# a-slide/Quade

Hardware: AMD Instinct MI355X
Metric: read-pairs/sec demultiplexed (2x150 bp, dual 8 bp index) (higher is better)
Workload: dtype u8

## Files before the change

quade_amd/csrc/quade_deflate.hip:

```cpp
#include <hip/hip_runtime.h>
#include <stdint.h>
#include <stdio.h>

#include "crc_lds.h"
#include "quade_deflate.h"

namespace {
constexpr int BLOCK = 256, TILE = BLOCK * 16;
constexpr uint32_t HEADER_BITS = 80 + 3 + 14 + 19 * 3 + 259 * 4;

__device__ uint32_t rev_bits(uint32_t v, int n) { return __brev(v) >> (32 - n); }

__device__ void code_lengths(const uint32_t* freq, int n, uint8_t* len, uint16_t* order , uint32_t* w , int16_t* parent ) {
    int m = 0;
    for (int s = 0; s < n; ++s) {
        len[s] = 0;
        if (freq[s]) order[m++] = (uint16_t)s;
    }
    for (int s = 0; m < 2 && s < n; ++s) {
        bool used = false;
        for (int i = 0; i < m; ++i) used |= order[i] == s;
        if (!used) order[m++] = (uint16_t)s;
    }
    auto f = [&](int s) -> uint32_t { return freq[s] ? freq[s] : 1u; };
    for (int i = 1; i < m; ++i) {
        const uint16_t s = order[i];
        int j = i - 1;
        while (j >= 0 && (f(order[j]) > f(s) || (f(order[j]) == f(s) && order[j] > s))) {
            order[j + 1] = order[j];
            --j;
        }
        order[j + 1] = s;
    }
    for (int i = 0; i < m; ++i) w[i] = f(order[i]);
    for (int i = 0; i < 2 * m - 1; ++i) parent[i] = -1;
    int leaf = 0, inner = m, next = m;
    while (next < 2 * m - 1) {
        int pick[2];
        for (int k = 0; k < 2; ++k) pick[k] = (leaf < m && (inner >= next || w[leaf] <= w[inner])) ? leaf++ : inner++;
        w[next] = w[pick[0]] + w[pick[1]];
        parent[pick[0]] = parent[pick[1]] = (int16_t)next;
        ++next;
    }
    int bl[16] = {0};
    w[2 * m - 2] = 0;
    for (int k = 2 * m - 3; k >= 0; --k) w[k] = w[parent[k]] + 1;
    for (int i = 0; i < m; ++i) ++bl[w[i] < 15 ? w[i] : 15];
    uint32_t kraft = 0;
    for (int d = 1; d <= 15; ++d) kraft += (uint32_t)bl[d] << (15 - d);
    for (uint32_t excess = kraft - (1u << 15); excess > 0; --excess) {
        int bits = 14;
        while (bl[bits] == 0) --bits;
        --bl[bits];
        bl[bits + 1] += 2;
        --bl[15];
    }
    int at = 0;
    for (int bits = 15; bits >= 1; --bits)
        for (int c = 0; c < bl[bits]; ++c) len[order[at++]] = (uint8_t)bits;
}

__global__ __launch_bounds__(BLOCK) void huff_pieces(const uint8_t* text, const qd_deflate_piece* pieces, uint8_t* out,
                                                     int64_t out_stride, uint32_t* out_bytes) {
    __shared__ uint32_t hist[4][4][256];
    __shared__ uint32_t freq[257];
    __shared__ uint32_t lut[257];
    __shared__ uint8_t len[257];
    __shared__ uint16_t order[257];
    __shared__ uint32_t wtmp[513];
    __shared__ int16_t parent[513];
    __shared__ uint32_t scan[BLOCK];
    __shared__ uint32_t words[TILE * 15 / 32 + 16];
    __shared__ uint32_t carry_word, carry_bits;
    const int tid = threadIdx.x, wave = tid >> 6, rep = tid & 3;
    const int64_t a = (int64_t)pieces[blockIdx.x].text_off, L = (int64_t)pieces[blockIdx.x].text_len;
    const uint8_t* src = text + a;
    uint32_t* dst = reinterpret_cast<uint32_t*>(out + (int64_t)blockIdx.x * out_stride);
    for (int i = tid; i < 4 * 4 * 256; i += BLOCK) (&hist[0][0][0])[i] = 0;
    __syncthreads();
    for (int64_t t = 0; t < L; t += TILE) {
        const int64_t p = t + (int64_t)tid * 16;
        if (p + 16 <= L) {
            const uint4 v = *reinterpret_cast<const uint4*>(src + p);
            const uint32_t q[4] = {v.x, v.y, v.z, v.w};
#pragma unroll
            for (int j = 0; j < 16; ++j) atomicAdd(&hist[wave][rep][(q[j >> 2] >> (8 * (j & 3))) & 0xff], 1u);
        } else {
            for (int64_t i = p; i < L; ++i) atomicAdd(&hist[wave][rep][src[i]], 1u);
        }
    }
    __syncthreads();
    for (int s = tid; s < 256; s += BLOCK) {
        uint32_t c = 0;
        for (int i = 0; i < 16; ++i) c += (&hist[0][0][0])[i * 256 + s];
        freq[s] = c;
    }
    if (tid == 0) freq[256] = 1;
    __syncthreads();
    if (tid == 0) {
        code_lengths(freq, 257, len, order, wtmp, parent);
        int blc[16] = {0}, nxt[16] = {0};
        for (int s = 0; s < 257; ++s) ++blc[len[s]];
        blc[0] = 0;
        for (int b = 1, c = 0; b <= 15; ++b) {
            c = (c + blc[b - 1]) << 1;
            nxt[b] = c;
        }
        for (int s = 0; s < 257; ++s) lut[s] = len[s] ? ((uint32_t)len[s] | (rev_bits((uint32_t)nxt[len[s]]++, len[s]) << 8)) : 0;
        uint64_t acc = 0;
        int cnt = 0, wi = 0;
        auto put = [&](uint32_t v, int n) {
            acc |= (uint64_t)v << cnt;
            cnt += n;
            if (cnt >= 32) {
                dst[wi++] = (uint32_t)acc;
                acc >>= 32;
                cnt -= 32;
            }
        };
        const uint8_t head[10] = {0x1f, 0x8b, 8, 0, 0, 0, 0, 0, 0, 0xff};
        for (int i = 0; i < 10; ++i) put(head[i], 8);
        put(1, 1);
        put(2, 2);
        put(0, 5);
        put(1, 5);
        put(15, 4);
        const uint8_t ord[19] = {16, 17, 18, 0, 8, 7, 9, 6, 10, 5, 11, 4, 12, 3, 13, 2, 14, 1, 15};
        for (int k = 0; k < 19; ++k) put(ord[k] < 16 ? 4 : 0, 3);
        for (int s = 0; s < 257; ++s) put(rev_bits(len[s], 4), 4);
        put(rev_bits(1, 4), 4);
        put(rev_bits(1, 4), 4);
        carry_word = (uint32_t)acc;
        carry_bits = (uint32_t)cnt;
        scan[0] = (uint32_t)wi;
        uint64_t bits = HEADER_BITS;
        for (int s = 0; s < 257; ++s) bits += (uint64_t)freq[s] * len[s];
        scan[1] = ((bits + 7) / 8 + 8 + 8 <= (uint64_t)out_stride) ? 1u : 0u;
    }
    __syncthreads();
    uint32_t out_word = scan[0];
    const bool fits = scan[1] != 0;
    __syncthreads();
    if (!fits) {
        if (tid == 0) out_bytes[blockIdx.x] = 0;
        return;
    }
    for (int64_t t = 0; t < L; t += TILE) {
        const int64_t p = t + (int64_t)tid * 16;
        uint32_t q[4] = {0, 0, 0, 0};
        int nbytes = 0;
        if (p + 16 <= L) {
            const uint4 v = *reinterpret_cast<const uint4*>(src + p);
            q[0] = v.x; q[1] = v.y; q[2] = v.z; q[3] = v.w;
            nbytes = 16;
        } else if (p < L) {
            nbytes = (int)(L - p);
            for (int i = 0; i < nbytes; ++i) q[i >> 2] |= (uint32_t)src[p + i] << (8 * (i & 3));
        }
        uint64_t b[4] = {0, 0, 0, 0};
        uint32_t nb = 0;
#pragma unroll
        for (int j = 0; j < 16; ++j) {
            if (j < nbytes) {
                const uint32_t e = lut[(q[j >> 2] >> (8 * (j & 3))) & 0xff];
                const uint64_t c = e >> 8;
                const uint32_t l = e & 0xff, wi = nb >> 6, sh = nb & 63;
                b[wi] |= c << sh;
                if (sh + l > 64 && wi < 3) b[wi + 1] |= c >> (64 - sh);
                nb += l;
            }
        }
        uint32_t x = nb;
#pragma unroll
        for (int d = 1; d < 64; d <<= 1) {
            const uint32_t y = __shfl_up(x, d, 64);
            if ((tid & 63) >= d) x += y;
        }
        if ((tid & 63) == 63) scan[wave] = x;
        __syncthreads();
        uint32_t base = 0, total = 0;
#pragma unroll
        for (int i = 0; i < BLOCK / 64; ++i) {
            const uint32_t v = scan[i];
            if (i < wave) base += v;
            total += v;
        }
        const uint32_t mine = base + x - nb;
        const uint32_t cb = carry_bits, cw = carry_word;
        const uint32_t nwords = (cb + total + 31) >> 5;
        for (uint32_t i = tid; i <= nwords; i += BLOCK) words[i] = i == 0 ? cw : 0;
        __syncthreads();
        if (nb) {
            const uint32_t pos = cb + mine, w0 = pos >> 5, sh = pos & 31;
            uint32_t prev = 0;
#pragma unroll
            for (int i = 0; i < 8; ++i) {
                const uint32_t d = (uint32_t)(b[i >> 1] >> (32 * (i & 1)));
                const uint32_t o = sh ? (d << sh) | (prev >> (32 - sh)) : d;
                if (o && 32u * i < nb + sh) atomicOr(&words[w0 + i], o);
                prev = d;
            }
            const uint32_t o = sh ? prev >> (32 - sh) : 0;
            if (o) atomicOr(&words[w0 + 8], o);
        }
        __syncthreads();
        const uint32_t full = (cb + total) >> 5;
        for (uint32_t i = tid; i < full; i += BLOCK) dst[out_word + i] = words[i];
        __syncthreads();
        if (tid == 0) {
            carry_word = words[full];
            carry_bits = (cb + total) & 31;
        }
        out_word += full;
        __syncthreads();
    }
    if (tid == 0) {
        uint64_t acc = carry_word;
        int cnt = (int)carry_bits;
        const uint32_t e = lut[256];
        acc |= (uint64_t)(e >> 8) << cnt;
        cnt += (int)(e & 0xff);
        uint8_t* bytes = reinterpret_cast<uint8_t*>(dst) + (size_t)out_word * 4;
        int nby = 0;
        while (cnt > 0) {
            bytes[nby++] = (uint8_t)acc;
            acc >>= 8;
            cnt -= 8;
        }
        const uint32_t c = pieces[blockIdx.x].crc32, isz = (uint32_t)L;
        for (int i = 0; i < 4; ++i) bytes[nby++] = (uint8_t)(c >> (8 * i));
        for (int i = 0; i < 4; ++i) bytes[nby++] = (uint8_t)(isz >> (8 * i));
        out_bytes[blockIdx.x] = out_word * 4 + (uint32_t)nby;
    }
}

}

hipError_t qd_launch_huffman(const uint8_t* text, const qd_deflate_piece* pieces, uint32_t n_pieces, uint8_t* out, int64_t out_stride,
                             uint32_t* out_bytes, hipStream_t st) {
    if (n_pieces == 0) return hipSuccess;
    hipLaunchKernelGGL(huff_pieces, dim3(n_pieces), dim3(BLOCK), 0, st, text, pieces, out, out_stride, out_bytes);
    return hipGetLastError();
}

namespace {
#ifndef QD_LZ_WAVES
#define QD_LZ_WAVES 8
#endif
constexpr int LZ_SUB = QD_LZ_SUB, LZ_WAVES = QD_LZ_WAVES, LZ_BLOCK = 64 * LZ_WAVES, LZ_REG = LZ_SUB / LZ_WAVES;
constexpr int LZ_HASH_BITS = 11, LZ_NICE = 32, LZ_DNA_MIN = 12, LZ_MATCH_BITS = 13, LZ_MAXLEN = 256;
constexpr int LZ_CRC_SW = LZ_WAVES >= 16 ? 17 : (LZ_WAVES >= 8 ? 33 : 65);
constexpr int LZ_TEXT_WORDS = (LZ_SUB + 320) / 4;
constexpr int LZ_NL = 286, LZ_ND = 30;
static_assert(LZ_SUB <= 65536 && LZ_SUB % 256 == 0, "table entries are 16-bit positions inside the sub-block");

__device__ __forceinline__ uint32_t rd32(const uint32_t* tw, uint32_t p) {
    const uint32_t i = p >> 2;
    return __builtin_amdgcn_alignbyte(tw[i + 1], tw[i], p & 3u);
}
__device__ __forceinline__ void rd256(const uint32_t* tw, uint32_t p, uint32_t (&a)[8]) {
    const uint32_t i = p >> 2, sh = p & 3u;
    uint32_t w[9];
#pragma unroll
    for (int k = 0; k < 9; ++k) w[k] = tw[i + k];
#pragma unroll
    for (int k = 0; k < 8; ++k) a[k] = __builtin_amdgcn_alignbyte(w[k + 1], w[k], sh);
}
__device__ __forceinline__ uint32_t same32(const uint32_t* tw, const uint32_t (&a)[8], uint32_t c) {
    uint32_t b[8];
    rd256(tw, c, b);
    uint32_t n = 32;
#pragma unroll
    for (int k = 7; k >= 0; --k) {
        const uint32_t x = a[k] ^ b[k];
        if (x) n = 4u * (uint32_t)k + ((uint32_t)__builtin_ctz(x) >> 3);
    }
    return n;
}
__device__ __forceinline__ bool bases4(uint32_t v) {
    return __builtin_amdgcn_perm(0x4E000000u, 0x47544341u, (v >> 1) & 0x07070707u) == v;
}
__device__ __forceinline__ void len_symbol(uint32_t l, uint32_t& sym, uint32_t& eb, uint32_t& ev) {
    if (l < 8) {
        sym = 257 + l;
        eb = ev = 0;
    } else if (l == 255) {
        sym = 285;
        eb = ev = 0;
    } else {
        const uint32_t n = 31u - (uint32_t)__clz(l);
        eb = n - 2;
        sym = 257 + 4 * (n - 1) + ((l >> eb) & 3u);
        ev = l & ((1u << eb) - 1);
    }
}
__device__ __forceinline__ void dist_symbol(uint32_t d, uint32_t& sym, uint32_t& eb, uint32_t& ev) {
    if (d < 4) {
        sym = d;
        eb = ev = 0;
    } else {
        const uint32_t n = 31u - (uint32_t)__clz(d);
        eb = n - 1;
        sym = 2 * n + ((d >> eb) & 1u);
        ev = d & ((1u << eb) - 1);
    }
}
__device__ __forceinline__ uint32_t len_extra_bits(uint32_t sym) {
    return (sym < 265 || sym == 285) ? 0u : (sym - 261) >> 2;
}
__device__ __forceinline__ uint32_t dist_extra_bits(uint32_t sym) { return sym < 4 ? 0u : (sym >> 1) - 1; }

__device__ void block_code_lengths(const uint32_t* freq, int n, uint8_t* len, uint32_t* fx, uint16_t* order, uint32_t* w, int16_t* parent,
                                   uint32_t* m_out) {
    __shared__ uint32_t bl[16];
    const int tid = threadIdx.x, nthr = blockDim.x;
    for (int s = tid; s < n; s += nthr) {
        fx[s] = freq[s];
        len[s] = 0;
    }
    if (tid < 16) bl[tid] = 0;
    if (tid == 0) *m_out = 0;
    __syncthreads();
    for (int s = tid; s < n; s += nthr)
        if (fx[s]) atomicAdd(m_out, 1u);
    __syncthreads();
    if (tid == 0 && *m_out < 2) {
        int used = (int)*m_out;
        for (int s = 0; used < 2 && s < n; ++s)
            if (!fx[s]) {
                fx[s] = 1;
                ++used;
            }
        *m_out = (uint32_t)used;
    }
    __syncthreads();
    const int m = (int)*m_out;
    for (int s = tid; s < n; s += nthr) {
        const uint32_t f = fx[s];
        if (!f) continue;
        int rank = 0;
        for (int t = 0; t < n; ++t) {
            const uint32_t g = fx[t];
            rank += (g != 0 && (g < f || (g == f && t < s))) ? 1 : 0;
        }
        order[rank] = (uint16_t)s;
        w[rank] = f;
    }
    for (int i = tid; i < 2 * m - 1; i += nthr) parent[i] = -1;
    __syncthreads();
    if (tid == 0) {
        int leaf = 0, inner = m, next = m;
        while (next < 2 * m - 1) {
            int pick[2];
            for (int k = 0; k < 2; ++k) pick[k] = (leaf < m && (inner >= next || w[leaf] <= w[inner])) ? leaf++ : inner++;
            w[next] = w[pick[0]] + w[pick[1]];
            parent[pick[0]] = parent[pick[1]] = (int16_t)next;
            ++next;
        }
    }
    __syncthreads();
    for (int i = tid; i < m; i += nthr) {
        uint32_t d = 0;
        for (int k = i; parent[k] >= 0; k = parent[k]) ++d;
        atomicAdd(&bl[d < 15 ? d : 15], 1u);
    }
    __syncthreads();
    if (tid == 0) {
        uint32_t kraft = 0;
        for (int d = 1; d <= 15; ++d) kraft += bl[d] << (15 - d);
        for (uint32_t excess = kraft - (1u << 15); excess > 0; --excess) {
            int bits = 14;
            while (bl[bits] == 0) --bits;
            --bl[bits];
            bl[bits + 1] += 2;
            --bl[15];
        }
    }
    __syncthreads();
    for (int i = tid; i < m; i += nthr) {
        int bits = 15;
        for (uint32_t upto = bl[15]; (uint32_t)i >= upto && bits > 1;) upto += bl[--bits];
        len[order[i]] = (uint8_t)bits;
    }
    __syncthreads();
}

__device__ void block_canonical_lut(const uint8_t* len, int n, uint32_t* lut) {
    __shared__ uint32_t cnt[16], nxt[16];
    const int tid = threadIdx.x, nthr = blockDim.x;
    if (tid < 16) cnt[tid] = 0;
    __syncthreads();
    for (int s = tid; s < n; s += nthr)
        if (len[s]) atomicAdd(&cnt[len[s]], 1u);
    __syncthreads();
    if (tid == 0) {
        uint32_t c = 0;
        for (int b = 1; b <= 15; ++b) {
            c = (c + (b > 1 ? cnt[b - 1] : 0u)) << 1;
            nxt[b] = c;
        }
    }
    __syncthreads();
    for (int s = tid; s < n; s += nthr) {
        const uint32_t l = len[s];
        uint32_t rank = 0;
        for (int t = 0; t < s; ++t) rank += len[t] == l ? 1u : 0u;
        lut[s] = l ? (l | (rev_bits(nxt[l] + rank, (int)l) << 8)) : 0u;
    }
    __syncthreads();
}

__device__ __forceinline__ void lds_barrier() { asm volatile("s_waitcnt lgkmcnt(0)\n\ts_barrier" ::: "memory"); }

#if defined(QD_LZ_TIMING)
__device__ unsigned long long g_lz_ticks[8];
#define LZ_STAMP(k)                                                          \
    do {                                                                     \
        __syncthreads();                                                     \
        const uint64_t now_ = (uint64_t)wall_clock64();                      \
        if (threadIdx.x == 0) atomicAdd(&g_lz_ticks[k], (unsigned long long)(now_ - since_)); \
        since_ = now_;                                                       \
    } while (0)
#else
#define LZ_STAMP(k) \
    do {            \
    } while (0)
#endif

__global__ __launch_bounds__(LZ_BLOCK) void lz_subblocks(const uint8_t* text, const qd_lz_sub* subs, uint32_t* tokens, uint8_t* sub_out,
                                                         int64_t sub_stride, uint32_t* sub_bytes, uint32_t* sub_crc) {
    extern __shared__ __attribute__((aligned(16))) uint8_t lz_lds[];
    uint32_t* tw = reinterpret_cast<uint32_t*>(lz_lds);
    uint32_t* table = reinterpret_cast<uint32_t*>(lz_lds + (size_t)LZ_TEXT_WORDS * 4);
    __shared__ uint32_t lfreq[288], dfreq[32], llut[288], dlut[32];
    __shared__ uint8_t llen[288], dlen[32], bcost[256];
    __shared__ uint32_t wave_ntok[LZ_WAVES], scan[LZ_WAVES], ctl[4];
    __shared__ uint32_t carry_word, carry_bits;
    const uint32_t tid = threadIdx.x, lane = tid & 63u, wave = tid >> 6;
    const uint32_t L = subs[blockIdx.x].text_len;
    const uint8_t* src = text + subs[blockIdx.x].text_off;
    uint32_t* dst = reinterpret_cast<uint32_t*>(sub_out + (int64_t)blockIdx.x * sub_stride);
    uint32_t* tok0 = tokens + (size_t)blockIdx.x * LZ_SUB;
#if defined(QD_LZ_TIMING)
    uint64_t since_ = (uint64_t)wall_clock64();
#endif

    static_assert((1u << LZ_HASH_BITS) == 8 * 256, "the byte histogram's replicas borrow the hash table's space");
    for (uint32_t i = tid; i < (1u << LZ_HASH_BITS); i += LZ_BLOCK) table[i] = 0;
    for (uint32_t i = tid; i < 288; i += LZ_BLOCK) lfreq[i] = 0;
    if (tid < 32) dfreq[tid] = 0;
    __syncthreads();
    for (uint32_t i = tid; i < (uint32_t)LZ_TEXT_WORDS / 4; i += LZ_BLOCK) {
        uint4 v = make_uint4(0, 0, 0, 0);
        const uint32_t b = i * 16;
        if (b + 16 <= L) {
            v = *reinterpret_cast<const uint4*>(src + b);
        } else if (b < L) {
            uint32_t q[4] = {0, 0, 0, 0};
            for (uint32_t k = b; k < L; ++k) q[(k - b) >> 2] |= (uint32_t)src[k] << (8 * ((k - b) & 3));
            v = make_uint4(q[0], q[1], q[2], q[3]);
        }
        reinterpret_cast<uint4*>(tw)[i] = v;
        if (b < L) {
            const uint32_t q[4] = {v.x, v.y, v.z, v.w}, nby = min(16u, L - b);
            uint32_t* rep = table + (tid & 7u);
#pragma unroll
            for (uint32_t k = 0; k < 16; ++k)
                if (k < nby) atomicAdd(&rep[((q[k >> 2] >> (8 * (k & 3))) & 0xFFu) << 3], 1u);
        }
    }
    __syncthreads();
    if (tid < 256) {
        uint32_t h = 0;
#pragma unroll
        for (int r = 0; r < 8; ++r) h += table[(tid << 3) + r];
        const int c = h ? (int)(__log2f((float)L / (float)h) + 0.5f) : 12;
        bcost[tid] = (uint8_t)(c < 1 ? 1 : (c > 12 ? 12 : c));
    }
    __syncthreads();
    LZ_STAMP(0);
    if (sub_crc) {
        static_assert((4u << LZ_HASH_BITS) >= 4096 + 64 && (size_t)LZ_BLOCK * LZ_CRC_SW * 4 >= (size_t)LZ_SUB, "the CRC stage's tables and slices");
        qdcrc::stage_tables<LZ_BLOCK>(table);
        __syncthreads();
        const uint32_t crc = qdcrc::crc32_lds<LZ_BLOCK, LZ_CRC_SW>(tw, L, table, table + 1024);
        if (tid == 0) sub_crc[blockIdx.x] = crc;
    }
    for (uint32_t i = tid; i < (1u << LZ_HASH_BITS); i += LZ_BLOCK) table[i] = 0;
    __syncthreads();
    LZ_STAMP(1);

    for (uint32_t r0 = 0; r0 < L; r0 += LZ_BLOCK) {
        const uint32_t p = r0 + tid;
        uint32_t ins_h = 0xFFFFFFFFu, ins_v = 0;
        if (p < L) {
            uint32_t a[8];
            rd256(tw, p, a);
            uint32_t best = 0, dist = 0;
            if (p + 4 <= L) {
                const uint32_t h = (a[0] * 2654435761u) >> (32 - LZ_HASH_BITS);
                const uint32_t bucket = table[h];
                if (p >= 1 && rd32(tw, p - 1) == a[0]) {
                    best = same32(tw, a, p - 1);
                    dist = 1;
                }
#pragma unroll
                for (int k = 0; k < 2; ++k) {
                    const uint32_t c = (bucket >> (16 * k)) & 0xFFFFu;
                    uint32_t n = 0;
                    if (c < p && rd32(tw, c) == a[0]) n = same32(tw, a, c);
                    if (c < p && p - c <= 32768u && n > best) {
                        best = n;
                        dist = p - c;
                    }
                }
                best = min(best, L - p);
                const uint32_t need = (bases4(a[0]) && bases4(a[1])) ? (uint32_t)LZ_DNA_MIN : 4u;
                if (best < need) {
                    best = 0;
                } else {
                    uint32_t c8 = 0;
#pragma unroll
                    for (int k = 0; k < 8; ++k) c8 += bcost[(a[k >> 2] >> (8 * (k & 3))) & 0xFFu];
                    const uint32_t mbits = (uint32_t)LZ_MATCH_BITS + (dist > 1 ? 31u - (uint32_t)__clz(dist) : 0u);
                    if (best * c8 < mbits * 8) best = 0;
                }
#if defined(QD_LZ_RACY)
                table[h] = (bucket << 16) | p;
#else
                ins_h = h;
                ins_v = (bucket << 16) | p;
#endif
            }
            tok0[p] = best | (dist << 8);
        }
        lds_barrier();
#if !defined(QD_LZ_RACY)
        if (ins_h != 0xFFFFFFFFu) atomicMax(&table[ins_h], ins_v);
        lds_barrier();
#endif
    }
    __syncthreads();

    LZ_STAMP(2);
    {
        const uint32_t rbeg = wave * LZ_REG, rend = min(rbeg + (uint32_t)LZ_REG, L);
        uint32_t* tok = tok0 + rbeg;
        uint32_t ntok = 0;
        int carry = 0;
        constexpr uint32_t AHEAD = (1u << LZ_HASH_BITS) / LZ_WAVES / 64;
        static_assert(AHEAD >= 1 && AHEAD * 64 * LZ_WAVES == (1u << LZ_HASH_BITS), "the waves' shares of the table's space");
        uint32_t* cbuf = table + wave * (AHEAD * 64);
        uint32_t in_buf = AHEAD;
        for (uint32_t base = rbeg; base < rend; base += 64) {
            const uint32_t p = base + lane;
            const int limit = (int)min(64u, rend - base);
            uint32_t eff = 0, dist = 0;
            if (in_buf == AHEAD) {
#pragma unroll
                for (uint32_t j = 0; j < AHEAD; ++j) cbuf[64 * j + lane] = p + 64 * j < rend ? tok0[p + 64 * j] : 0u;
                in_buf = 0;
            }
            const uint32_t cd = cbuf[64 * in_buf + lane];
            ++in_buf;
            if ((int)lane < limit) {
                eff = min(cd & 0xFFu, rend - p);
                dist = cd >> 8;
                if (eff < 4) eff = 0;
            }
            const uint32_t lit = (tw[p >> 2] >> (8 * (p & 3u))) & 0xFFu;
            const uint32_t eff_next = (uint32_t)__shfl_down((int)eff, 1, 64);
            const bool deferred = eff != 0 && (int)lane + 1 < limit && eff_next > eff && eff < (uint32_t)LZ_NICE;
            const uint64_t mm = __ballot(eff != 0 && !deferred);
            const uint64_t xm = __ballot(eff >= (uint32_t)LZ_NICE && !deferred);
            uint32_t tlen = eff;
            const uint32_t tdist = dist;
            uint64_t starts = 0;
            int s = carry;
            while (s < limit) {
                if ((mm >> s) & 1ull) {
                    uint32_t len = (uint32_t)__builtin_amdgcn_readlane((int)eff, s);
                    if ((xm >> s) & 1ull) {
                        const uint32_t D = (uint32_t)__builtin_amdgcn_readlane((int)dist, s);
                        const uint32_t ps = base + (uint32_t)s;
                        const uint32_t x = rd32(tw, ps + 4 * lane) ^ rd32(tw, ps - D + 4 * lane);
                        const uint64_t nz = __ballot(x != 0);
                        len = LZ_MAXLEN;
                        if (nz) {
                            const int fl = __builtin_ctzll(nz);
                            const uint32_t xf = (uint32_t)__builtin_amdgcn_readlane((int)x, fl);
                            len = 4u * (uint32_t)fl + ((uint32_t)__builtin_ctz(xf) >> 3);
                        }
                        len = min(len, rend - ps);
                        if ((int)lane == s) tlen = len;
                    }
                    starts |= 1ull << s;
                    s += (int)len;
                } else {
                    const uint64_t rest = (mm >> s) << s;
                    int nxt = rest ? __builtin_ctzll(rest) : 64;
                    if (nxt > limit) nxt = limit;
                    const uint64_t upto = nxt >= 64 ? ~0ull : ((1ull << nxt) - 1);
                    starts |= upto & ~((1ull << s) - 1);
                    s = nxt;
                }
            }
            if (!((mm >> lane) & 1ull)) tlen = 0;
            carry = s - 64;
            if ((starts >> lane) & 1ull) {
                uint32_t t;
                if (tlen) {
                    t = (tlen - 3) | ((tdist - 1) << 8);
                    uint32_t sym, eb, ev;
                    len_symbol(tlen - 3, sym, eb, ev);
                    atomicAdd(&lfreq[sym], 1u);
                    dist_symbol(tdist - 1, sym, eb, ev);
                    atomicAdd(&dfreq[sym], 1u);
                } else {
                    t = 0x80000000u | lit;
                    atomicAdd(&lfreq[lit], 1u);
                }
                tok[ntok + (uint32_t)__popcll(starts & ((1ull << lane) - 1))] = t;
            }
            ntok += (uint32_t)__popcll(starts);
        }
        if (lane == 0) wave_ntok[wave] = ntok;
    }
    if (tid == 0) lfreq[256] = 1;
    __syncthreads();
    LZ_STAMP(3);

    {
        uint32_t* fx = tw;
        uint16_t* order = reinterpret_cast<uint16_t*>(tw + 288);
        uint32_t* w = tw + 288 + 144;
        int16_t* parent = reinterpret_cast<int16_t*>(tw + 288 + 144 + 576);
        block_code_lengths(lfreq, LZ_NL, llen, fx, order, w, parent, &ctl[2]);
        block_code_lengths(dfreq, LZ_ND, dlen, fx, order, w, parent, &ctl[2]);
    }
    LZ_STAMP(4);
    uint32_t* words = tw + 2048;
    block_canonical_lut(llen, LZ_NL, llut);
    block_canonical_lut(dlen, LZ_ND, dlut);
    if (tid == 0) ctl[3] = 0;
    __syncthreads();
    {
        uint32_t bits = 0;
        for (uint32_t s = tid; s < (uint32_t)LZ_NL; s += LZ_BLOCK) bits += lfreq[s] * (llen[s] + (s > 256 ? len_extra_bits(s) : 0u));
        for (uint32_t s = tid; s < (uint32_t)LZ_ND; s += LZ_BLOCK) bits += dfreq[s] * (dlen[s] + dist_extra_bits(s));
        if (bits) atomicAdd(&ctl[3], bits);
    }
    __syncthreads();
    LZ_STAMP(7);
    if (tid == 0) {
        int nl = LZ_NL, nd = LZ_ND;
        while (nl > 257 && llen[nl - 1] == 0) --nl;
        while (nd > 1 && dlen[nd - 1] == 0) --nd;
        uint64_t acc = 0;
        int cnt = 0, wi = 0;
        auto put = [&](uint32_t v, int n) {
            acc |= (uint64_t)v << cnt;
            cnt += n;
            if (cnt >= 32) {
                dst[wi++] = (uint32_t)acc;
                acc >>= 32;
                cnt -= 32;
            }
        };
        put(0, 1);
        put(2, 2);
        put((uint32_t)(nl - 257), 5);
        put((uint32_t)(nd - 1), 5);
        put(15, 4);
        const uint8_t ord[19] = {16, 17, 18, 0, 8, 7, 9, 6, 10, 5, 11, 4, 12, 3, 13, 2, 14, 1, 15};
        for (int k = 0; k < 19; ++k) put(ord[k] == 0 ? 2u : ((ord[k] == 17 || ord[k] == 18) ? 3u : 5u), 3);
        auto len_at = [&](int i) -> uint32_t { return i < nl ? llen[i] : dlen[i - nl]; };
        auto put_len = [&](uint32_t v) { put(rev_bits(15u + v, 5), 5); };
        const int nseq = nl + nd;
        for (int i = 0; i < nseq;) {
            const uint32_t v = len_at(i);
            int run = 1;
            while (i + run < nseq && len_at(i + run) == v) ++run;
            i += run;
            if (v == 0) {
                while (run >= 11) {
                    const int r = run < 138 ? run : 138;
                    put(6, 3);
                    put((uint32_t)(r - 11), 7);
                    run -= r;
                }
                if (run >= 3) {
                    put(2, 3);
                    put((uint32_t)(run - 3), 3);
                    run = 0;
                }
                for (; run > 0; --run) put(0, 2);
            } else {
                put_len(v);
                --run;
                while (run >= 3) {
                    const int r = run < 6 ? run : 6;
                    put_len(16);
                    put((uint32_t)(r - 3), 2);
                    run -= r;
                }
                for (; run > 0; --run) put_len(v);
            }
        }
        carry_word = (uint32_t)acc;
        carry_bits = (uint32_t)cnt;
        const uint64_t bits = 3 + 14 + 19 * 3 + 5 * (uint64_t)(nl + nd) + ctl[3];
        ctl[0] = (uint32_t)wi;
        ctl[1] = ((bits + 7) / 8 + 3 + 4 + 8 <= (uint64_t)sub_stride) ? 1u : 0u;
    }
    __syncthreads();
    LZ_STAMP(5);
    uint32_t out_word = ctl[0];
    if (ctl[1] == 0) {
        if (tid == 0) sub_bytes[blockIdx.x] = 0;
        return;
    }
    constexpr int LZ_TPL = 4;
    uint32_t pre[LZ_WAVES + 1];
    pre[0] = 0;
#pragma unroll
    for (int i = 0; i < LZ_WAVES; ++i) pre[i + 1] = pre[i] + wave_ntok[i];
    const uint32_t T = pre[LZ_WAVES];
    for (uint32_t g0 = 0; g0 < T; g0 += LZ_BLOCK * LZ_TPL) {
        uint32_t t[LZ_TPL];
#pragma unroll
        for (int j = 0; j < LZ_TPL; ++j) {
            const uint32_t g = g0 + tid * LZ_TPL + j;
            t[j] = 0;
            if (g < T) {
                uint32_t wv = 0;
#pragma unroll
                for (int i = 1; i < LZ_WAVES; ++i) wv += g >= pre[i] ? 1u : 0u;
                t[j] = tok0[(size_t)wv * LZ_REG + (g - pre[wv])];
            }
        }
        uint64_t b[LZ_TPL];
        uint32_t nb[LZ_TPL], mine = 0;
#pragma unroll
        for (int j = 0; j < LZ_TPL; ++j) {
            b[j] = 0;
            nb[j] = 0;
            if (g0 + tid * LZ_TPL + j < T) {
                if (t[j] & 0x80000000u) {
                    const uint32_t e = llut[t[j] & 0xFFu];
                    b[j] = e >> 8;
                    nb[j] = e & 0xFFu;
                } else {
                    uint32_t sym, eb, ev;
                    len_symbol(t[j] & 0xFFu, sym, eb, ev);
                    uint32_t e = llut[sym];
                    b[j] = (uint64_t)(e >> 8) | ((uint64_t)ev << (e & 0xFFu));
                    nb[j] = (e & 0xFFu) + eb;
                    dist_symbol((t[j] >> 8) & 0x7FFFu, sym, eb, ev);
                    e = dlut[sym];
                    b[j] |= ((uint64_t)(e >> 8) | ((uint64_t)ev << (e & 0xFFu))) << nb[j];
                    nb[j] += (e & 0xFFu) + eb;
                }
            }
            mine += nb[j];
        }
        uint32_t x = mine;
#pragma unroll
        for (int d = 1; d < 64; d <<= 1) {
            const uint32_t y = __shfl_up(x, d, 64);
            if (lane >= (uint32_t)d) x += y;
        }
        if (lane == 63) scan[wave] = x;
        lds_barrier();
        uint32_t before = 0, total = 0;
#pragma unroll
        for (int i = 0; i < LZ_WAVES; ++i) {
            const uint32_t v = scan[i];
            if ((uint32_t)i < wave) before += v;
            total += v;
        }
        const uint32_t cb = carry_bits, cw = carry_word;
        const uint32_t nwords = (cb + total + 31) >> 5;
        for (uint32_t i = tid; i <= nwords + 2; i += LZ_BLOCK) words[i] = i == 0 ? cw : 0;
        lds_barrier();
        uint32_t pos = cb + before + x - mine;
#pragma unroll
        for (int j = 0; j < LZ_TPL; ++j) {
            if (nb[j]) {
                const uint32_t w0 = pos >> 5, sh = pos & 31u;
                const uint64_t lo = b[j] << sh;
                const uint32_t hi = sh ? (uint32_t)(b[j] >> (64 - sh)) : 0u;
                if ((uint32_t)lo) atomicOr(&words[w0], (uint32_t)lo);
                if ((uint32_t)(lo >> 32)) atomicOr(&words[w0 + 1], (uint32_t)(lo >> 32));
                if (hi) atomicOr(&words[w0 + 2], hi);
            }
            pos += nb[j];
        }
        lds_barrier();
        const uint32_t full = (cb + total) >> 5;
        for (uint32_t i = tid; i < full; i += LZ_BLOCK) dst[out_word + i] = words[i];
        if (tid == 0) {
            carry_word = words[full];
            carry_bits = (cb + total) & 31u;
        }
        out_word += full;
    }
    __syncthreads();
    LZ_STAMP(6);
    if (tid == 0) {
        uint64_t acc = carry_word;
        int cnt = (int)carry_bits;
        const uint32_t e = llut[256];
        acc |= (uint64_t)(e >> 8) << cnt;
        cnt += (int)(e & 0xFFu);
        cnt += 3;
        uint8_t* bytes = reinterpret_cast<uint8_t*>(dst) + (size_t)out_word * 4;
        int nby = 0;
        while (cnt > 0) {
            bytes[nby++] = (uint8_t)acc;
            acc >>= 8;
            cnt -= 8;
        }
        bytes[nby++] = 0;
        bytes[nby++] = 0;
        bytes[nby++] = 0xFF;
        bytes[nby++] = 0xFF;
        sub_bytes[blockIdx.x] = out_word * 4 + (uint32_t)nby;
    }
}

__global__ __launch_bounds__(256) void lz_members(const qd_deflate_piece* pieces, const qd_lz_sub* subs, const uint32_t* first_sub, uint32_t n_subs,
                                                  const uint8_t* sub_out, int64_t sub_stride, const uint32_t* sub_bytes, uint8_t* out,
                                                  int64_t out_stride, uint32_t* out_bytes) {
    const bool empty = blockIdx.x >= n_subs;
    const uint32_t piece = empty ? blockIdx.x - n_subs : subs[blockIdx.x].piece;
    const uint32_t j0 = first_sub[piece], j1 = first_sub[piece + 1], j = blockIdx.x;
    if (empty && j1 != j0) return;
    uint64_t total = 10 + 2 + 8, off = 10;
    bool ok = true;
    for (uint32_t k = j0; k < j1; ++k) {
        const uint32_t n = sub_bytes[k];
        ok = ok && n > 0;
        total += n;
        if (k < j) off += n;
    }
    const bool first = empty || j == j0, last = empty || j + 1 == j1;
    if (!ok || total > (uint64_t)out_stride) {
        if (first && threadIdx.x == 0) out_bytes[piece] = 0;
        return;
    }
    uint8_t* dst = out + (int64_t)piece * out_stride;
    if (!empty) {
        const uint32_t n = sub_bytes[j];
        const uint8_t* s = sub_out + (int64_t)j * sub_stride;
        for (uint32_t k = threadIdx.x; k < n; k += 256) dst[off + k] = s[k];
        off += n;
    }
    if (threadIdx.x == 0) {
        if (first) {
            const uint8_t head[10] = {0x1f, 0x8b, 8, 0, 0, 0, 0, 0, 0, 0xff};
            for (int i = 0; i < 10; ++i) dst[i] = head[i];
        }
        if (last) {
            dst[off++] = 0x03;
            dst[off++] = 0x00;
            const uint32_t c = pieces[piece].crc32, isz = pieces[piece].text_len;
            for (int i = 0; i < 4; ++i) dst[off++] = (uint8_t)(c >> (8 * i));
            for (int i = 0; i < 4; ++i) dst[off++] = (uint8_t)(isz >> (8 * i));
            out_bytes[piece] = (uint32_t)off;
        }
    }
}
}

hipError_t qd_launch_lz_subblocks(const uint8_t* text, const qd_lz_sub* subs, uint32_t n_subs, uint32_t* tokens, uint8_t* sub_out, int64_t sub_stride,
                                  uint32_t* sub_bytes, uint32_t* sub_crc, hipStream_t st) {
    if (n_subs == 0) return hipSuccess;
    constexpr size_t lds = (size_t)LZ_TEXT_WORDS * 4 + (4u << LZ_HASH_BITS);
    static_assert(LZ_TEXT_WORDS % 4 == 0, "the text is staged 16 bytes at a time");
    hipError_t e = hipFuncSetAttribute(reinterpret_cast<const void*>(lz_subblocks), hipFuncAttributeMaxDynamicSharedMemorySize, (int)lds);
    if (e != hipSuccess) return e;
    hipLaunchKernelGGL(lz_subblocks, dim3(n_subs), dim3(LZ_BLOCK), lds, st, text, subs, tokens, sub_out, sub_stride, sub_bytes, sub_crc);
#if defined(QD_LZ_TIMING)
    {
        unsigned long long t[8];
        (void)hipStreamSynchronize(st);
        (void)hipMemcpyFromSymbol(t, HIP_SYMBOL(g_lz_ticks), sizeof t);
        static const char* names[8] = {"stage+histogram", "crc", "candidates", "parse", "code lengths", "header (one lane)", "encode", "tables"};
        unsigned long long sum = 0;
        for (int k = 0; k < 8; ++k) sum += t[k];
        fprintf(stderr, "lz_subblocks phases (all launches so far, %u sub-blocks in this one):", n_subs);
        for (int k = 0; k < 8; ++k) fprintf(stderr, " %s %.1f %%", names[k], sum ? 100.0 * (double)t[k] / (double)sum : 0.0);
        fprintf(stderr, "\n");
    }
#endif
    return hipGetLastError();
}

hipError_t qd_launch_lz_members(const qd_deflate_piece* pieces, uint32_t n_pieces, const qd_lz_sub* subs, const uint32_t* first_sub, uint32_t n_subs,
                                const uint8_t* sub_out, int64_t sub_stride, const uint32_t* sub_bytes, uint8_t* out, int64_t out_stride, uint32_t* out_bytes,
                                hipStream_t st) {
    if (n_pieces == 0) return hipSuccess;
    hipLaunchKernelGGL(lz_members, dim3(n_subs + n_pieces), dim3(256), 0, st, pieces, subs, first_sub, n_subs, sub_out, sub_stride, sub_bytes,
                       out, out_stride, out_bytes);
    return hipGetLastError();
}

hipError_t qd_launch_lz(const uint8_t* text, const qd_deflate_piece* pieces, uint32_t n_pieces, const qd_lz_sub* subs, const uint32_t* first_sub,
                        uint32_t n_subs, uint32_t* tokens, uint8_t* sub_out, int64_t sub_stride, uint32_t* sub_bytes, uint8_t* out,
                        int64_t out_stride, uint32_t* out_bytes, hipStream_t st) {
    if (n_pieces == 0) return hipSuccess;
    const hipError_t e = qd_launch_lz_subblocks(text, subs, n_subs, tokens, sub_out, sub_stride, sub_bytes, nullptr, st);
    if (e != hipSuccess) return e;
    return qd_launch_lz_members(pieces, n_pieces, subs, first_sub, n_subs, sub_out, sub_stride, sub_bytes, out, out_stride, out_bytes, st);
}
```

Before: 178.8 billion.

## Parallelize dynamic Huffman header emission across the block with ballots and scans

The serial single-thread loop that wrote the DEFLATE dynamic-block header (trimmed code-length runs, RLE codes 16/17/18) is replaced by a block-parallel version. Table trimming uses wave ballots, run starts are marked as ballot bitmasks in LDS, each thread derives its symbol's run position and emitted bits, and a wave-plus-block prefix scan places the bits via atomicOr into LDS words. The constant code-length-code lengths are folded into a compile-time word. This removes a long single-lane critical section per sub-block, at the cost of extra barriers, LDS atomics and more intricate run-splitting logic that must match the serial encoder exactly.

```diff
diff --git a/quade_amd/csrc/quade_deflate.hip b/quade_amd/csrc/quade_deflate.hip
--- a/quade_amd/csrc/quade_deflate.hip
+++ b/quade_amd/csrc/quade_deflate.hip
@@ -408,6 +408,13 @@
         lut[s] = l ? (l | (rev_bits(nxt[l] + rank, (int)l) << 8)) : 0u;
     }
     __syncthreads();
+}
+
+constexpr uint64_t lz_clc_lengths() {
+    const uint8_t ord[19] = {16, 17, 18, 0, 8, 7, 9, 6, 10, 5, 11, 4, 12, 3, 13, 2, 14, 1, 15};
+    uint64_t c = 0;
+    for (int k = 0; k < 19; ++k) c |= (uint64_t)(ord[k] == 0 ? 2u : ((ord[k] == 17 || ord[k] == 18) ? 3u : 5u)) << (3 * k);
+    return c;
 }
 
 __device__ __forceinline__ void lds_barrier() { asm volatile("s_waitcnt lgkmcnt(0)\n\ts_barrier" ::: "memory"); }
@@ -652,66 +659,109 @@
     }
     __syncthreads();
     LZ_STAMP(7);
-    if (tid == 0) {
-        int nl = LZ_NL, nd = LZ_ND;
-        while (nl > 257 && llen[nl - 1] == 0) --nl;
-        while (nd > 1 && dlen[nd - 1] == 0) --nd;
-        uint64_t acc = 0;
-        int cnt = 0, wi = 0;
-        auto put = [&](uint32_t v, int n) {
-            acc |= (uint64_t)v << cnt;
-            cnt += n;
-            if (cnt >= 32) {
-                dst[wi++] = (uint32_t)acc;
-                acc >>= 32;
-                cnt -= 32;
-            }
-        };
-        put(0, 1);
-        put(2, 2);
-        put((uint32_t)(nl - 257), 5);
-        put((uint32_t)(nd - 1), 5);
-        put(15, 4);
-        const uint8_t ord[19] = {16, 17, 18, 0, 8, 7, 9, 6, 10, 5, 11, 4, 12, 3, 13, 2, 14, 1, 15};
-        for (int k = 0; k < 19; ++k) put(ord[k] == 0 ? 2u : ((ord[k] == 17 || ord[k] == 18) ? 3u : 5u), 3);
-        auto len_at = [&](int i) -> uint32_t { return i < nl ? llen[i] : dlen[i - nl]; };
-        auto put_len = [&](uint32_t v) { put(rev_bits(15u + v, 5), 5); };
-        const int nseq = nl + nd;
-        for (int i = 0; i < nseq;) {
-            const uint32_t v = len_at(i);
-            int run = 1;
-            while (i + run < nseq && len_at(i + run) == v) ++run;
-            i += run;
-            if (v == 0) {
-                while (run >= 11) {
-                    const int r = run < 138 ? run : 138;
-                    put(6, 3);
-                    put((uint32_t)(r - 11), 7);
-                    run -= r;
+    {
+        __shared__ uint32_t hmask[2 * 5];
+        const uint64_t lused = __ballot(lane < (uint32_t)(LZ_NL - 257) && llen[257 + lane] != 0);
+        const uint64_t dused = __ballot(lane < (uint32_t)LZ_ND && dlen[lane] != 0);
+        const uint32_t nl = 257u + (lused ? 64u - (uint32_t)__builtin_clzll(lused) : 0u);
+        const uint32_t nd = dused ? 64u - (uint32_t)__builtin_clzll(dused) : 1u;
+        const uint32_t nseq = nl + nd;
+        static_assert(LZ_NL + LZ_ND < 5 * 64, "the runs' start flags: five waves' ballots, with room for the end's");
+        auto len_at = [&](uint32_t i) -> uint32_t { return i < nl ? llen[i] : dlen[i - nl]; };
+        for (uint32_t i = tid; i < 5 * 64; i += LZ_BLOCK) {
+            const bool start = i < nseq && (i == 0 || len_at(i) != len_at(i - 1));
+            const uint64_t m = __ballot(start || i == nseq);
+            if (lane == 0) {
+                hmask[2 * (i >> 6)] = (uint32_t)m;
+                hmask[2 * (i >> 6) + 1] = (uint32_t)(m >> 32);
+            }
+        }
+        constexpr uint32_t HWORDS = (3 + 14 + 19 * 3 + 5 * (LZ_NL + LZ_ND) + 31) / 32 + 2;
+        for (uint32_t i = tid; i < HWORDS; i += LZ_BLOCK) words[i] = 0;
+        lds_barrier();
+        if (tid == 0) {
+            constexpr uint64_t clc = lz_clc_lengths();
+            const uint64_t lo = (uint64_t)((2u << 1) | ((nl - 257u) << 3) | ((nd - 1u) << 8) | (15u << 13)) | (clc << 17);
+            atomicOr(&words[0], (uint32_t)lo);
+            atomicOr(&words[1], (uint32_t)(lo >> 32));
+            atomicOr(&words[2], (uint32_t)(clc >> 47));
+        }
+        uint32_t hbits = 3 + 14 + 19 * 3;
+        for (uint32_t i0 = 0; i0 < nseq; i0 += LZ_BLOCK) {
+            const uint32_t i = i0 + tid;
+            uint32_t bits = 0, nb = 0;
+            if (i < nseq) {
+                uint32_t wi = i >> 5, m = hmask[wi] & (0xFFFFFFFFu >> (31u - (i & 31u)));
+                while (m == 0) m = hmask[--wi];
+                const uint32_t beg = 32u * wi + 31u - (uint32_t)__clz(m);
+                wi = i >> 5;
+                m = hmask[wi] & (0xFFFFFFFEu << (i & 31u));
+                while (m == 0) m = hmask[++wi];
+                const uint32_t end = 32u * wi + (uint32_t)__builtin_ctz(m);
+                const uint32_t v = len_at(i);
+                const uint32_t piece = v == 0 ? 138u : 6u, least = v == 0 ? 11u : 3u;
+                const uint32_t run = end - beg - (v == 0 ? 0u : 1u), whole = run / piece * piece;
+                const uint32_t one = v == 0 ? 0u : rev_bits(15u + v, 5), one_bits = v == 0 ? 2u : 5u;
+                if (v != 0 && i == beg) {
+                    bits = one;
+                    nb = one_bits;
+                } else {
+                    const uint32_t j = i - beg - (v == 0 ? 0u : 1u);
+                    const uint32_t at = j < whole ? j % piece : j - whole, r = j < whole ? piece : run - whole;
+                    if (r >= least) {
+                        if (at == 0) {
+                            if (v != 0) {
+                                bits = 31u | ((r - 3u) << 5);
+                                nb = 7;
+                            } else if (r >= 11u) {
+                                bits = 6u | ((r - 11u) << 3);
+                                nb = 10;
+                            }
+                        }
+                    } else if (v == 0 && r >= 3u) {
+                        if (at == 0) {
+                            bits = 2u | ((r - 3u) << 3);
+                            nb = 6;
+                        }
+                    } else {
+                        bits = one;
+                        nb = one_bits;
+                    }
                 }
-                if (run >= 3) {
-                    put(2, 3);
-                    put((uint32_t)(run - 3), 3);
-                    run = 0;
-                }
-                for (; run > 0; --run) put(0, 2);
-            } else {
-                put_len(v);
-                --run;
-                while (run >= 3) {
-                    const int r = run < 6 ? run : 6;
-                    put_len(16);
-                    put((uint32_t)(r - 3), 2);
-                    run -= r;
-                }
-                for (; run > 0; --run) put_len(v);
-            }
-        }
-        carry_word = (uint32_t)acc;
-        carry_bits = (uint32_t)cnt;
-        const uint64_t bits = 3 + 14 + 19 * 3 + 5 * (uint64_t)(nl + nd) + ctl[3];
-        ctl[0] = (uint32_t)wi;
-        ctl[1] = ((bits + 7) / 8 + 3 + 4 + 8 <= (uint64_t)sub_stride) ? 1u : 0u;
+            }
+            uint32_t x = nb;
+#pragma unroll
+            for (int d = 1; d < 64; d <<= 1) {
+                const uint32_t y = __shfl_up(x, d, 64);
+                if (lane >= (uint32_t)d) x += y;
+            }
+            if (lane == 63) scan[wave] = x;
+            lds_barrier();
+            uint32_t before = 0, total = 0;
+#pragma unroll
+            for (int k = 0; k < LZ_WAVES; ++k) {
+                const uint32_t s = scan[k];
+                if ((uint32_t)k < wave) before += s;
+                total += s;
+            }
+            if (nb) {
+                const uint32_t pos = hbits + before + x - nb;
+                const uint64_t lo = (uint64_t)bits << (pos & 31u);
+                if ((uint32_t)lo) atomicOr(&words[pos >> 5], (uint32_t)lo);
+                if ((uint32_t)(lo >> 32)) atomicOr(&words[(pos >> 5) + 1], (uint32_t)(lo >> 32));
+            }
+            hbits += total;
+            lds_barrier();
+        }
+        const uint32_t full = hbits >> 5;
+        for (uint32_t i = tid; i < full; i += LZ_BLOCK) dst[i] = words[i];
+        if (tid == 0) {
+            carry_word = words[full];
+            carry_bits = hbits & 31u;
+            const uint64_t bits = 3 + 14 + 19 * 3 + 5 * (uint64_t)(nl + nd) + ctl[3];
+            ctl[0] = full;
+            ctl[1] = ((bits + 7) / 8 + 3 + 4 + 8 <= (uint64_t)sub_stride) ? 1u : 0u;
+        }
     }
     __syncthreads();
     LZ_STAMP(5);
@@ -886,7 +936,7 @@
         unsigned long long t[8];
         (void)hipStreamSynchronize(st);
         (void)hipMemcpyFromSymbol(t, HIP_SYMBOL(g_lz_ticks), sizeof t);
-        static const char* names[8] = {"stage+histogram", "crc", "candidates", "parse", "code lengths", "header (one lane)", "encode", "tables"};
+        static const char* names[8] = {"stage+histogram", "crc", "candidates", "parse", "code lengths", "header", "encode", "tables"};
         unsigned long long sum = 0;
         for (int k = 0; k < 8; ++k) sum += t[k];
         fprintf(stderr, "lz_subblocks phases (all launches so far, %u sub-blocks in this one):", n_subs);
```

After: 178.6 billion. No clear change (-0.1%).
